# wangxb29/PPST

Hardware: AMD Instinct MI355X
Metric: 512x512 portrait swaps/sec/GPU (higher is better)
Workload: dtype bf16x3 (fp32 split into hi+lo bf16, 3 MFMA passes, fp32 accumulate); 1 GPU; simple_swapping 512x512 batch=8 per GPU, generator+encoders forward only (BASELINE configs[1]); image_parallel=1 batch per rank, no data-path collective

## Files before the change

include/ppst_hip.h:

```cpp
#ifndef PPST_HIP_H
#define PPST_HIP_H

#include <stddef.h>
#include <stdint.h>

#ifdef __cplusplus
extern "C" {
#endif

#define PPST_OK 0
#define PPST_EINVAL (-1)
#define PPST_EUNSUPPORTED (-2)
#define PPST_ENULL (-3)

enum { PPST_F32 = 0, PPST_F16 = 1, PPST_BF16 = 2, PPST_F64 = 3  };

enum { PPST_PAD_ZERO = 0, PPST_PAD_REFLECT = 1, PPST_PAD_REPLICATE = 2 };

enum { PPST_ACT_NONE = 0, PPST_ACT_LRELU = 1 , PPST_ACT_PRELU = 2 };

#define PPST_ABI_VERSION 3
int ppst_version(void);

#define PPST_ST_F32 0
// ... 73 lines not shown

typedef struct ppst_conv_args {
  const void* x;
  const void* wpack;
  const void* steps;
  void* y;
  const void* bias;
  const void* noise;
  const void* prelu;
  void* stats;
  const void* residual;
  float noise_weight;
  float out_scale;
  int32_t B, in_h, in_w, in_ld;
  int32_t out_h, out_w, out_ld, cout;
  int32_t nsteps, n_groups;
  int32_t pad_mode;
  int32_t in_off_y, in_off_x;
  int32_t out_sy, out_sx;
  int32_t act;
  int32_t precision;
  int32_t res_ld;
  int32_t tile_h, tile_w;
  int32_t halo;
  int32_t bn;
  const void* in_scale_shift;
  const void* in_prelu;
  int32_t in_c, in_act;
  int32_t flop_steps;
  int32_t tile_rows;
  int32_t a_slots;
  int32_t early_a;
  int32_t variant;
  int32_t reserved0;
  int32_t dual_b;
  int32_t io_st;
  int32_t k64;
  const void* in_res;
  int32_t in_res_ld;
  int32_t ksplit;
  const int32_t* ksplit_starts;
  void* ksplit_scratch;
  unsigned* ksplit_flags;
  uint32_t ksplit_epoch;
} ppst_conv_args;

int ppst_conv2d_mfma(const ppst_conv_args* a, void* stream);
int64_t ppst_conv_pack_wino_bytes(int cout, int cin);
int ppst_conv_pack_wino(const void* w, int64_t sn, int64_t sc, int64_t sy, int64_t sx, float scale, int cout, int cin,
                        void* out, void* stream);
int ppst_conv2d_f32(const ppst_conv_args* a, const void* w, int64_t sn, int64_t sc, int64_t sy, int64_t sx, float wscale,
                    const int32_t* src_c, const int32_t* src_ky, const int32_t* src_kx, void* stream);
int ppst_conv_tiles(int tile_h, int tile_w, int tile_rows);

int ppst_conv1x1_small_cin(const void* x, const void* w, const void* bias, void* y,
                           int64_t npix, int cin, int in_ld, int cout, float wscale,
                           int act, void* stream);
int ppst_conv1x1_small_cin_st(const void* x, const void* w, const void* bias, void* y,
                              int64_t npix, int cin, int in_ld, int cout, float wscale,
                              int act, int y_st , void* stream);
int ppst_conv1x1_small_cout(const void* x, const void* w, const void* bias, void* y,
                            int64_t npix, int cin, int cout, float wscale, void* stream);
int ppst_conv1x1_small_cout_st(const void* x, const void* w, const void* bias, void* y,
                               int64_t npix, int cin, int cout, float wscale, int x_st , void* stream);
int ppst_torgb_apply_st(const void* x, const void* scale_shift, const void* res, int res_ld, float out_scale, const void* w,
                        const void* bias, void* y, int B, int H, int W, int cin, float wscale, int x_st, void* stream);

int ppst_in_stats(const void* x, void* partial, int B, int H, int W, int C, int ld,
                  int rep_pad, int* n_partials, void* stream);
int ppst_in_finalize(const void* partial, int n_partials, const void* style,
                     int style_ld ,
                     const void* post_bias ,
                     void* scale_shift , int B, int C, double count,
                     float eps, void* stream);
int ppst_affine_act(const void* x, const void* scale_shift, const void* res,
                    const void* res_scale_shift , void* y,
                    int B, int64_t hw, int C, int x_ld, int res_ld, int y_ld,
                    int act , const void* prelu,
                    float out_scale,
                    int res_up2_w ,
                    void* stream);
int ppst_affine_act_st(const void* x, const void* scale_shift, const void* res, const void* res_scale_shift, void* y,
                       int B, int64_t hw, int C, int x_ld, int res_ld, int y_ld, int act, const void* prelu,
                       float out_scale, int res_up2_w, int x_st, int y_st, void* stream);
int ppst_affine_act_stats(const void* x, const void* scale_shift, const void* res,
                          const void* res_scale_shift, void* y, void* partial,
                          int B, int H, int W, int C, int x_ld, int res_ld, int y_ld,
                          int act, const void* prelu, float out_scale, int rep_pad,
                          int res_up2 , void* stream);
int ppst_upsample_nearest2(const void* x, void* y, int B, int H, int W, int C, void* stream);
int ppst_upsample_nearest2_st(const void* x, void* y, int B, int H, int W, int C, int st, void* stream);

int64_t ppst_gap_gmp_ws(int B, int64_t hw, int C);
int ppst_gap_gmp(const void* x, const void* mask, void* out, void* ws, int B, int H, int W,
                 int C, int ld, void* stream);
int ppst_gap_gmp_st(const void* x, const void* mask, void* out, void* ws, int B, int H, int W,
                    int C, int ld, int x_st, void* stream);
#define PPST_GROUP_MAX 32
typedef struct {
  const void* x;
  const void* mask;
  void* out;
  int32_t H, W, C, ld;
} ppst_gap_gmp_level;
int64_t ppst_gap_gmp_multi_level_ws(const ppst_gap_gmp_level* levels, int n, int B);
int ppst_gap_gmp_multi_level(const ppst_gap_gmp_level* levels, int n, int B, void* ws, int x_st, void* stream);
// ... 185 lines not shown
```

ppst_amd/_lib.py:

```python
import ctypes
import os

import torch

HERE = os.path.dirname(os.path.abspath(__file__))
LIB_PATH = os.environ.get("PPST_HIP_LIB") or os.path.join(HERE, "libppst_hip.so")

if not os.path.exists(LIB_PATH):
    raise ImportError(
        "ppst_amd: %s is missing -- build it with `python -m ppst_amd.build` "
        "(hipcc --offload-arch=gfx950). There is no CPU fallback." % LIB_PATH)

lib = ctypes.CDLL(LIB_PATH)

vp, i32, i64, f32, f64 = ctypes.c_void_p, ctypes.c_int, ctypes.c_int64, ctypes.c_float, ctypes.c_double


class PackJob(ctypes.Structure):
    _fields_ = [("w", vp), ("sn", i64), ("sc", i64), ("sy", i64), ("sx", i64), ("src_c", vp), ("src_ky", vp), ("src_kx", vp),
                ("out", vp), ("total", i64), ("block0", i64), ("scale", f32), ("cout", i32), ("bn", i32), ("nsteps", i32),
                ("n_groups", i32), ("x3", i32), ("f16", i32), ("nblocks", i32), ("dual", i32)]


class UpscaleJob(ctypes.Structure):
# ... 12 lines not shown
class LerpProblem(ctypes.Structure):
    _fields_ = [("a", vp), ("b", vp), ("y", vp), ("n", i64), ("r", f32)]


class GapGmpLevel(ctypes.Structure):
    _fields_ = [("x", vp), ("mask", vp), ("out", vp), ("H", i32), ("W", i32), ("C", i32), ("ld", i32)]


GROUP_MAX = 32


class ConvArgs(ctypes.Structure):
    _fields_ = [
        ("x", vp), ("wpack", vp), ("steps", vp), ("y", vp), ("bias", vp), ("noise", vp),
        ("prelu", vp), ("stats", vp), ("residual", vp),
        ("noise_weight", f32), ("out_scale", f32),
        ("B", i32), ("in_h", i32), ("in_w", i32), ("in_ld", i32),
        ("out_h", i32), ("out_w", i32), ("out_ld", i32), ("cout", i32),
        ("nsteps", i32), ("n_groups", i32), ("pad_mode", i32),
        ("in_off_y", i32), ("in_off_x", i32), ("out_sy", i32), ("out_sx", i32),
        ("act", i32), ("precision", i32), ("res_ld", i32), ("tile_h", i32), ("tile_w", i32),
        ("halo", i32), ("bn", i32), ("in_scale_shift", vp), ("in_prelu", vp), ("in_c", i32), ("in_act", i32),
        ("flop_steps", i32), ("tile_rows", i32), ("a_slots", i32), ("early_a", i32), ("variant", i32), ("reserved0", i32), ("dual_b", i32), ("io_st", i32), ("k64", i32),
        ("in_res", vp), ("in_res_ld", i32), ("ksplit", i32), ("ksplit_starts", vp),
        ("ksplit_scratch", vp), ("ksplit_flags", vp), ("ksplit_epoch", ctypes.c_uint32),
    ]


_SIGS = {
    "ppst_version": (i32, []),
    "ppst_guided_filter_tune": (i32, [i32, i32]),
    "ppst_upfirdn2d": (i32, [vp, vp, vp] + [i32] * 14 + [i32, vp]),
    "ppst_blur_nhwc": (i32, [vp, vp, vp] + [i32] * 10 + [vp, i32, vp]),
    "ppst_blur_nhwc_st": (i32, [vp, vp, vp] + [i32] * 10 + [vp, i32, i32, vp]),
    "ppst_fused_bias_act": (i32, [vp, vp, vp, vp, i64, i32, i32, i32, i32, f32, f32, i32, vp]),
    "ppst_nchw_to_nhwc": (i32, [vp, vp, i32, i32, i32, i32, vp]),
    "ppst_nhwc_to_nchw": (i32, [vp, vp, i32, i32, i32, i32, vp]),
    "ppst_conv_pack": (i32, [vp, i64, i64, i64, i64, f32, i32, i32, vp, vp, vp, i32, i32, i32, vp, vp]),
    "ppst_conv_pack_k64": (i32, [vp, i64, i64, i64, i64, f32, i32, i32, vp, vp, vp, i32, i32, i32, i32, vp, vp]),
    "ppst_conv_pack_up9_bytes": (i64, [i32, i32]),
    "ppst_conv_pack_up9": (i32, [vp, i64, i64, i64, i64, f32, i32, i32, vp, vp]),
    "ppst_conv_pack_wino_bytes": (i64, [i32, i32]),
    "ppst_conv_pack_wino": (i32, [vp, i64, i64, i64, i64, f32, i32, i32, vp, vp]),
    "ppst_conv_pack_dual": (i32, [vp, i64, i64, i64, i64, f32, i32, vp, vp, vp, i32, i32, i32, vp, vp]),
    "ppst_upscale_weight": (i32, [vp, vp, i32, i32, f32, vp]),
    "ppst_dgrad_s2d_stack_weight": (i32, [vp, vp, i32, i32, vp]),
    "ppst_depth_to_space_st": (i32, [vp, vp, i32, i32, i32, i32, i32, i32, i32, vp]),
    "ppst_pack_job_blocks": (i32, [i64]),
    "ppst_conv_pack_batch": (i32, [vp, i32, i32, vp]),
    "ppst_upscale_weight_batch": (i32, [vp, i32, i32, vp]),
    "ppst_conv2d_mfma": (i32, [ctypes.POINTER(ConvArgs), vp]),
    "ppst_conv2d_f32": (i32, [ctypes.POINTER(ConvArgs), vp, i64, i64, i64, i64, f32, vp, vp, vp, vp]),
    "ppst_conv_tiles": (i32, [i32, i32, i32]),
    "ppst_conv1x1_small_cin": (i32, [vp, vp, vp, vp, i64, i32, i32, i32, f32, i32, vp]),
    "ppst_conv1x1_small_cin_st": (i32, [vp, vp, vp, vp, i64, i32, i32, i32, f32, i32, i32, vp]),
    "ppst_conv1x1_small_cout": (i32, [vp, vp, vp, vp, i64, i32, i32, f32, vp]),
    "ppst_conv1x1_small_cout_st": (i32, [vp, vp, vp, vp, i64, i32, i32, f32, i32, vp]),
    "ppst_torgb_apply_st": (i32, [vp, vp, vp, i32, f32, vp, vp, vp, i32, i32, i32, i32, f32, i32, vp]),
    "ppst_in_stats": (i32, [vp, vp, i32, i32, i32, i32, i32, i32, ctypes.POINTER(i32), vp]),
    "ppst_in_finalize": (i32, [vp, i32, vp, i32, vp, vp, i32, i32, f64, f32, vp]),
    "ppst_affine_act": (i32, [vp, vp, vp, vp, vp, i32, i64, i32, i32, i32, i32, i32, vp, f32, i32, vp]),
    "ppst_affine_act_st": (i32, [vp, vp, vp, vp, vp, i32, i64, i32, i32, i32, i32, i32, vp, f32, i32, i32, i32, vp]),
    "ppst_affine_act_stats": (i32, [vp, vp, vp, vp, vp, vp, i32, i32, i32, i32, i32, i32, i32, i32, vp, f32, i32, i32, vp]),
    "ppst_upsample_nearest2": (i32, [vp, vp, i32, i32, i32, i32, vp]),
    "ppst_upsample_nearest2_st": (i32, [vp, vp, i32, i32, i32, i32, i32, vp]),
    "ppst_gap_gmp_ws": (i64, [i32, i64, i32]),
    "ppst_gap_gmp": (i32, [vp, vp, vp, vp, i32, i32, i32, i32, i32, vp]),
    "ppst_gap_gmp_st": (i32, [vp, vp, vp, vp, i32, i32, i32, i32, i32, i32, vp]),
    "ppst_avgpool": (i32, [vp, vp, i32, i32, i32, i32, i32, i32, i32, vp]),
    "ppst_bilinear": (i32, [vp, vp, i32, i32, i32, i32, i32, i32, i32, i32, vp]),
    "ppst_head_tail": (i32, [vp, vp, vp, vp, vp] + [i32] * 10 + [vp]),
    "ppst_maxpool2": (i32, [vp, vp, i32, i32, i32, i32, vp]),
    "ppst_linear": (i32, [vp, vp, vp, vp, i32, i32, i32, f32, f32, i32, i32, vp]),
    "ppst_l2norm_rows": (i32, [vp, vp, i32, i32, f32, i32, vp]),
    "ppst_lerp": (i32, [vp, vp, vp, i64, f32, vp]),
    "ppst_linear_grouped": (i32, [vp, i32, vp]),
    "ppst_l2norm_rows_grouped": (i32, [vp, i32, vp]),
    "ppst_lerp_grouped": (i32, [vp, i32, vp]),
    "ppst_gap_gmp_multi_level_ws": (i64, [vp, i32, i32]),
    "ppst_gap_gmp_multi_level": (i32, [vp, i32, i32, vp, i32, vp]),
    "ppst_spatial_modulation": (i32, [vp, vp, vp, vp, i32, i64, i32, vp]),
    "ppst_spatial_modulation_st": (i32, [vp, vp, vp, vp, i32, i64, i32, i32, vp]),
    "ppst_rselfcorr": (i32, [vp, vp, i32, i32, i32, i32, i32, vp]),
    "ppst_corr_prep": (i32, [vp, vp, i32, i32, i32, i32, vp]),
    "ppst_gemm_nt_f32": (i32, [vp, vp, vp, i32, i32, i32, i32, f32, vp]),
    "ppst_gemm_nn_f32": (i32, [vp, vp, vp, i32, i32, i32, i32, i32, i32, vp]),
    "ppst_unfold_rows": (i32, [vp, vp, i32, i32, i32, i32, i32, vp]),
    "ppst_unfold_rows_bwd": (i32, [vp, vp, i32, i32, i32, i32, i32, vp]),
    "ppst_gemm_nt_split": (i32, [vp, vp, vp, i32, i32, i32, i32, f32, i32, vp]),
    "ppst_gemm_nn_split": (i32, [vp, vp, vp, i32, i32, i32, i32, i32, i32, i32, vp]),
    "ppst_softmax_rows": (i32, [vp, i64, i32, f32, vp]),
    "ppst_unfold_patches": (i32, [vp, vp, i32, i32, i32, i32, i32, vp]),
    "ppst_fold_patches": (i32, [vp, vp, i32, i32, i32, i32, i32, vp]),
    "ppst_tensor2im_u8": (i32, [vp, vp, i32, i32, i32, i32, vp]),
    "ppst_resample_u8": (i32, [vp, vp, i32, i32, i32, i32, i32, i32, vp, vp, i32, vp]),
    "ppst_u8_to_tensor": (i32, [vp, vp, i32, i32, i32, i32, f32, f32, vp]),
    "ppst_resample_f32": (i32, [vp, vp, i32, i32, i32, i32, i32, vp, vp, i32, vp, vp, i32, i32, f32, f32, vp]),
    "ppst_png_bound": (i64, [i32, i32, i32]),
    "ppst_png_ws": (i64, [i32, i32, i32, i32]),
    "ppst_png_encode": (i32, [vp, vp, vp, i32, i32, i32, i32, vp, vp]),
    "ppst_lpips_pack_floats": (i64, []),
    "ppst_lpips_pack": (i32, [vp, vp, vp, vp, vp, vp, vp]),
    "ppst_lpips_dims": (i32, [i32, i32, ctypes.POINTER(i32)]),
    "ppst_lpips_ws": (i64, [i32, i32, i32]),
    "ppst_lpips_trunk": (i32, [vp, vp, ctypes.POINTER(i64), i32, vp, ctypes.POINTER(i64), i32, i32, i32, vp, vp]),
    "ppst_lpips_feature": (i32, [vp, i32, i32, i32, i32, vp, vp]),
# ... 89 lines not shown
```

ppst_amd/csrc/conv_wino.hip:

```cpp
#include "common.h"

struct WinoKArgs {
  const float* x;
  const unsigned char* wpack;
  const int4* steps;
  float* y;
  const float* bias;
  const float* noise;
  const float* prelu;
  float* stats;
  const float* residual;
  float noise_weight, out_scale;
  int B, in_h, in_w, in_ld, out_ld, cout, nchunk, pad_mode, act, res_ld;
  int tiles_y, tiles_x, n_tiles;
  const float* in_ss;
  const float* in_prelu;
  int in_c, in_act;
  KSplitDev ks;
};

__device__ __forceinline__ int wino_pad_index(int i, int n, int mode) {
  if (mode == PPST_PAD_REFLECT) {
    if (i < 0) i = -i;
    if (i >= n) i = 2 * (n - 1) - i;
  }
  return i < 0 ? 0 : (i >= n ? n - 1 : i);
}

#define WINO_LDA(dst, off) dst = *(const bf16x8*)(smem + (off))
#define WINO_MFMA(a_, b_, c_) c_ = __builtin_amdgcn_mfma_f32_16x16x32_bf16(a_, b_, c_, 0, 0, 0)
#define WINO_STEP_BYTES 8192
#define WINO_OOB ((int)0x80000000)

__device__ __forceinline__ void wino_split4(float4 v, uint2& hi, uint2& lo) {
  const unsigned h0 = f2bf_pk((ppst_f2){v.x, v.y}), h1 = f2bf_pk((ppst_f2){v.z, v.w});
  const float rx = v.x - __uint_as_float(h0 << 16), ry = v.y - __uint_as_float(h0 & 0xffff0000u);
  const float rz = v.z - __uint_as_float(h1 << 16), rw = v.w - __uint_as_float(h1 & 0xffff0000u);
  hi = make_uint2(h0, h1);
  lo = make_uint2(f2bf_pk((ppst_f2){rx, ry}), f2bf_pk((ppst_f2){rz, rw}));
}

__device__ __forceinline__ float wino_swap1(float v) {
  return __int_as_float(__builtin_amdgcn_update_dpp(0, __float_as_int(v), 0x128, 0xF, 0xF, true));
}

__device__ __forceinline__ int wino_lane() {
  int l = __builtin_amdgcn_mbcnt_hi(~0u, __builtin_amdgcn_mbcnt_lo(~0u, 0u));
  asm volatile("" : "+v"(l));
  return l;
}

template <int INMODE, bool KS = false>
__global__ __launch_bounds__(512, 2) void conv_wino_kernel(WinoKArgs a) {
  constexpr bool INSS = INMODE != 0;
  constexpr int NWV = 8, NTH = 64 * NWV, NTW = 4;
  constexpr int NRND = 3;
  constexpr int NP = 8, HH = 18;
  constexpr int PLANE = HH * NP * 16;
  constexpr int XIB = 8 * PLANE;
  constexpr int ABUF = 4 * XIB + 128;
  constexpr int TROW = 36;
  constexpr int TXI = 128 * TROW;
  constexpr int TBUF = 4 * TXI;
  __shared__ __attribute__((aligned(256))) unsigned char smem[2 * ABUF + 1024 * 2 * 4];
  float* const ss_lds = (float*)(smem + 2 * ABUF);

  const int nwg = gridDim.x;
  int wid;
  {
    int id = blockIdx.x, q = nwg >> 3, r = nwg & 7, xcd = id & 7;
    wid = (xcd < r ? xcd * (q + 1) : r * (q + 1) + (xcd - r) * q) + (id >> 3);
  }
  const int m_count = a.B * a.tiles_y * a.tiles_x;
  const int ntile = wid / m_count;
  int midx = wid - ntile * m_count;
  const int b = midx / (a.tiles_y * a.tiles_x);
  midx -= b * a.tiles_y * a.tiles_x;
  const int tyi = midx / a.tiles_x, txi = midx - tyi * a.tiles_x;
  const int ty0 = tyi * 16, tx0 = txi * 16;

  const int tid = threadIdx.x, lane = tid & 63, wave = __builtin_amdgcn_readfirstlane(tid >> 6);
  const int xi = wave >> 1, nh = wave & 1;
  const int r16 = lane & 15, g = lane >> 4;

#if defined(__HIP_DEVICE_COMPILE__)
  typedef const __attribute__((address_space(4))) int4* StepPtr;
#else
  typedef const int4* StepPtr;
#endif
  StepPtr steps = (StepPtr)a.steps;
  int nchunk = a.nchunk, c0 = 0;
  if (KS && a.ks.S > 1) {
    int s0, s1;
    ks_range(a.ks, (int)blockIdx.y, s0, s1);
    c0 = s0 / 9;
    nchunk = s1 / 9 - c0;
    steps += c0 * 9;
  }
  const int nsteps = nchunk * 3;
  const int64_t xoff_ = (int64_t)b * a.in_h * a.in_w * a.in_ld;
  const float* xb = a.x + (((int64_t)__builtin_amdgcn_readfirstlane((int)(xoff_ >> 32)) << 32) | (unsigned)__builtin_amdgcn_readfirstlane((int)xoff_));

  const int sp = lane & 7, se = (lane >> 3) & 1, sg = lane >> 4;
  int colA, colB;
  bool okA, okB;
  {
    auto col = [&](int k, bool& ok) __attribute__((always_inline)) {
      int ix = tx0 + 2 * sp - 1 + k;
      ok = (ix >= 0 && ix < a.in_w) || a.pad_mode != PPST_PAD_ZERO;
      ix = wino_pad_index(ix, a.in_w, a.pad_mode);
      return ok ? (ix * a.in_ld + sg * 8) * 4 : WINO_OOB;
    };
    colA = col(se ? 3 : 0, okA);
    colB = col(se ? 1 : 2, okB);
  }
  const bool interior = a.pad_mode != PPST_PAD_ZERO || (ty0 >= 1 && ty0 + 16 < a.in_h && tx0 >= 1 && tx0 + 16 < a.in_w);
  int rowoff[NRND];
#pragma unroll
  for (int r = 0; r < NRND; ++r) {
    const int hrow = wave + NWV * r;
    int iy = ty0 + hrow - 1;
    const bool inb = iy >= 0 && iy < a.in_h;
    int o = -1;
    if (hrow < HH && (inb || a.pad_mode != PPST_PAD_ZERO)) {
      iy = wino_pad_index(iy, a.in_h, a.pad_mode);
      o = iy * a.in_w * a.in_ld * 4;
    }
    rowoff[r] = __builtin_amdgcn_readfirstlane(o);
  }
  const __amdgpu_buffer_rsrc_t xrs = __builtin_amdgcn_make_buffer_rsrc((void*)xb, 0, a.in_h * a.in_w * a.in_ld * 4, 0x00020000);
  const float in_slope = (INSS && a.in_act == PPST_ACT_PRELU && a.in_prelu) ? a.in_prelu[0] : 0.f;
  const float in_neg = !INSS ? 1.f : a.in_act == PPST_ACT_LRELU ? 0.2f : a.in_act == PPST_ACT_PRELU ? in_slope : 1.f;
  const float in_pos = (INSS && a.in_act == PPST_ACT_LRELU) ? 1.41421356237309515f : 1.f;
  auto in_act = [&](float t) __attribute__((always_inline)) -> float { return (t > 0.f ? t : t * in_neg) * in_pos; };
  float4 rd[4];
  auto stage_load = [&](float4 (&q)[4], int r, int chan) __attribute__((always_inline)) {
    const int so = (rowoff[r] >= 0 ? rowoff[r] : 0) + chan * 4;
    const int va = (INMODE == 0 && rowoff[r] < 0) ? WINO_OOB : colA, vb = (INMODE == 0 && rowoff[r] < 0) ? WINO_OOB : colB;
    q[0] = __builtin_bit_cast(float4, __builtin_amdgcn_raw_buffer_load_b128(xrs, va, so, 0));
    q[1] = __builtin_bit_cast(float4, __builtin_amdgcn_raw_buffer_load_b128(xrs, va, so + 16, 0));
    q[2] = __builtin_bit_cast(float4, __builtin_amdgcn_raw_buffer_load_b128(xrs, vb, so, 0));
    q[3] = __builtin_bit_cast(float4, __builtin_amdgcn_raw_buffer_load_b128(xrs, vb, so + 16, 0));
  };
  auto stage_skip = [&](int r) __attribute__((always_inline)) { return r == NRND - 1 && wave >= 2; };
  const int chan_first = steps[0].x;
  auto stage_prep = [&](float4 (&q)[4], int r, int chan, int part) __attribute__((always_inline)) {
    const bool rowok = rowoff[r] >= 0;
    if (INSS) {
      const float4* p = (const float4*)((const unsigned char*)ss_lds + (chan - chan_first) * 8 + (wino_lane() >> 4) * 64) + part * 2;
      const float4 s0 = p[0], s1 = p[1];
      auto nact = [&](float t) __attribute__((always_inline)) -> float { return INMODE == 2 ? in_act(t) : t; };
      if (interior) {
#pragma unroll
        for (int h = part; h < 4; h += 2) {
          float4 v = q[h];
          v.x = nact(s0.x * v.x + s0.y); v.y = nact(s0.z * v.y + s0.w);
          v.z = nact(s1.x * v.z + s1.y); v.w = nact(s1.z * v.w + s1.w);
          q[h] = v;
        }
      } else {
#pragma unroll
        for (int h = part; h < 4; h += 2) {
          float4 v = q[h];
          if (rowok && (h < 2 ? okA : okB)) {
            v.x = nact(s0.x * v.x + s0.y); v.y = nact(s0.z * v.y + s0.w);
            v.z = nact(s1.x * v.z + s1.y); v.w = nact(s1.z * v.w + s1.w);
          } else v = make_float4(0.f, 0.f, 0.f, 0.f);
          q[h] = v;
        }
      }
    }
  };
  auto stage_put = [&](float4 (&q)[4], int r, int slot, int piece) __attribute__((always_inline)) {
    const int hrow = wave + NWV * r;
    const float4 A0 = q[0], A1 = q[1], B0_ = q[2], B1_ = q[3];
    float4 V0, V1;
    int i;
    const int ln = wino_lane(), se = (ln >> 3) & 1, stb = (ln >> 4) * PLANE + (ln & 7) * 16;
    const float sgn = se ? -1.f : 1.f;
    if (piece == 0) {
      i = se ? 3 : 0;
      V0 = make_float4(A0.x - B0_.x, A0.y - B0_.y, A0.z - B0_.z, A0.w - B0_.w);
      V1 = make_float4(A1.x - B1_.x, A1.y - B1_.y, A1.z - B1_.z, A1.w - B1_.w);
    } else {
      i = se ? 2 : 1;
      V0 = make_float4(wino_swap1(B0_.x) + sgn * B0_.x, wino_swap1(B0_.y) + sgn * B0_.y, wino_swap1(B0_.z) + sgn * B0_.z, wino_swap1(B0_.w) + sgn * B0_.w);
      V1 = make_float4(wino_swap1(B1_.x) + sgn * B1_.x, wino_swap1(B1_.y) + sgn * B1_.y, wino_swap1(B1_.z) + sgn * B1_.z, wino_swap1(B1_.w) + sgn * B1_.w);
    }
    uint2 h0, l0, h1, l1;
    wino_split4(V0, h0, l0);
    wino_split4(V1, h1, l1);
    unsigned char* dst = smem + (slot * ABUF + hrow * NP * 16) + i * XIB + stb;
    *(uint4*)dst = make_uint4(h0.x, h0.y, h1.x, h1.y);
    *(uint4*)(dst + 4 * PLANE) = make_uint4(l0.x, l0.y, l1.x, l1.y);
  };

  const int64_t woff_ = ((((int64_t)ntile * 4 + xi) * 2 + nh) * (a.nchunk * 3) + c0 * 3) * WINO_STEP_BYTES;
  const unsigned char* wbase = a.wpack + (((int64_t)__builtin_amdgcn_readfirstlane((int)(woff_ >> 32)) << 32) |
                                          (unsigned)__builtin_amdgcn_readfirstlane((int)woff_));
  const __amdgpu_buffer_rsrc_t wrs = __builtin_amdgcn_make_buffer_rsrc((void*)wbase, 0, nsteps * WINO_STEP_BYTES, 0x00020000);
  bf16x8 B0[2][2], B1[2][2];
  auto load_b = [&](bf16x8 (&dst)[2][2], int s, int half) __attribute__((always_inline)) {
    const int so = s * WINO_STEP_BYTES + half * 4096;
    const int lo16 = wino_lane() * 16;
#pragma unroll
    for (int n = 0; n < 2; ++n)
#pragma unroll
      for (int h = 0; h < 2; ++h)
        dst[n][h] = __builtin_bit_cast(bf16x8, __builtin_amdgcn_raw_buffer_load_b128(wrs, lo16 + (n * 2 + h) * 1024, so, 0));
  };

  load_b(B0, 0, 0); load_b(B1, 0, 1);
  {
    float4 q[NRND][4];
#pragma unroll
    for (int r = 0; r < NRND; ++r) stage_load(q[r], r, chan_first);
    if (INSS) {
      const float* src = a.in_ss + ((int64_t)b * a.in_c + chan_first) * 2;
      for (int i = tid * 4; i < nchunk * 64; i += NTH * 4) *(float4*)(ss_lds + i) = *(const float4*)(src + i);
      __syncthreads();
    }
#pragma unroll
    for (int r = 0; r < NRND; ++r) {
      if (!stage_skip(r)) {
        stage_prep(q[r], r, chan_first, 0); stage_prep(q[r], r, chan_first, 1);
        stage_put(q[r], r, 0, 0); stage_put(q[r], r, 0, 1);
      }
    }
  }
  asm volatile("s_waitcnt lgkmcnt(0)\n\ts_barrier" ::: "memory");

  f32x4 acc[8][NTW];
#pragma unroll
  for (int i = 0; i < 8; ++i)
#pragma unroll
    for (int j = 0; j < NTW; ++j) acc[i][j] = (f32x4){0.f, 0.f, 0.f, 0.f};

#define WA_OFF(slot, dy, mt) ((slot) * ABUF + xi * XIB + g * PLANE + ((2 * (mt) + (dy)) * NP + r16) * 16)
  int s = 0;
  for (int c = 0; c < nchunk; ++c) {
    const int slot = c & 1;
    const bool more = c + 1 < nchunk;
    const int chan_next = steps[(more ? c + 1 : c) * 9].x;
    const int aoff0 = WA_OFF(slot, 0, 0);
    int aoff1 = aoff0;
    asm volatile("" : "+v"(aoff1));
    bf16x8 ah = *(const bf16x8*)(smem + aoff0);
    bf16x8 al = *(const bf16x8*)(smem + aoff0 + 4 * PLANE);
#pragma unroll
    for (int dy = 0; dy < 3; ++dy) {
      const int sn = s + 1 < nsteps ? s + 1 : s;
      stage_load(rd, dy, chan_next);
      __builtin_amdgcn_sched_barrier(0);
#pragma unroll
      for (int mt = 0; mt < 8; ++mt) {
        bf16x8 nh_, nl_;
        if (mt < 7) {
          WINO_LDA(nh_, aoff0 + (2 * (mt + 1) + dy) * NP * 16);
          WINO_LDA(nl_, aoff0 + (2 * (mt + 1) + dy) * NP * 16 + 4 * PLANE);
        } else {
          WINO_LDA(nh_, aoff1 + dy * NP * 16);
          WINO_LDA(nl_, aoff1 + dy * NP * 16 + 4 * PLANE);
        }
        __builtin_amdgcn_sched_barrier(0);
#pragma unroll
        for (int n = 0; n < 2; ++n) {
          WINO_MFMA(al, B0[n][0], acc[mt][n]);
          WINO_MFMA(ah, B0[n][1], acc[mt][n]);
          WINO_MFMA(ah, B0[n][0], acc[mt][n]);
        }
        ah = nh_;
        al = nl_;
      }
      __builtin_amdgcn_sched_barrier(0);
      load_b(B0, sn, 0);
      __builtin_amdgcn_sched_barrier(0);
      const bool skip = stage_skip(dy);
#pragma unroll
      for (int mt = 0; mt < 8; ++mt) {
        bf16x8 nh_ = ah, nl_ = al;
        if (mt < 7) {
          WINO_LDA(nh_, aoff1 + (2 * (mt + 1) + dy) * NP * 16);
          WINO_LDA(nl_, aoff1 + (2 * (mt + 1) + dy) * NP * 16 + 4 * PLANE);
        } else if (dy < 2) {
          WINO_LDA(nh_, aoff0 + (dy + 1) * NP * 16);
          WINO_LDA(nl_, aoff0 + (dy + 1) * NP * 16 + 4 * PLANE);
        }
        __builtin_amdgcn_sched_barrier(0);
        if (!skip) {
          if (mt == 2) stage_prep(rd, dy, chan_next, 0);
          if (mt == 3) stage_prep(rd, dy, chan_next, 1);
          if (mt == 4) stage_put(rd, dy, slot ^ 1, 0);
          if (mt == 6) stage_put(rd, dy, slot ^ 1, 1);
        }
#pragma unroll
        for (int n = 0; n < 2; ++n) {
          WINO_MFMA(al, B1[n][0], acc[mt][2 + n]);
          WINO_MFMA(ah, B1[n][1], acc[mt][2 + n]);
          WINO_MFMA(ah, B1[n][0], acc[mt][2 + n]);
        }
        ah = nh_;
        al = nl_;
      }
      __builtin_amdgcn_sched_barrier(0);
      load_b(B1, sn, 1);
      __builtin_amdgcn_sched_barrier(0);
      ++s;
    }
    asm volatile("s_waitcnt lgkmcnt(0)\n\ts_barrier" ::: "memory");
  }
#undef WA_OFF

  if (KS && a.ks.S > 1) {
    const int S = a.ks.S, y = (int)blockIdx.y;
    float* const slot0 = a.ks.scratch + (int64_t)wid * (S - 1) * (8 * NTW * 4 * NTH) + tid;
    if (y < S - 1) {
      float* const dst = slot0 + (int64_t)y * (8 * NTW * 4 * NTH);
      KS_SCATTER(acc, 8, NTW, NTH, dst)
      ks_publish(a.ks, wid, y, tid);
      return;
    }
    ks_wait(a.ks, wid, tid);
    KS_GATHER(acc, 8, NTW, NTH, S, slot0);
  }

  float* const T = (float*)smem;
  float* const red = (float*)smem;
  const int act = a.act & 0xff;
  const bool res_after = (a.act >> 8) & 1;
  const float slope = (act == PPST_ACT_PRELU && a.prelu) ? a.prelu[0] : 0.f;
  constexpr int NML = NTH / 32, NIT = 32 / NML;
  const int f32_ = tid & 31, mloc = tid >> 5;
  const int n0 = ntile * 128 + f32_ * 4;
  const bool nok = n0 < a.cout;
  const int64_t img = (int64_t)b * a.in_h * a.in_w;
  float* const yb = a.y + img * a.out_ld;
  const float* const nzb = a.noise ? a.noise + img : nullptr;
  const float* const rb = a.residual ? a.residual + img * a.res_ld : nullptr;
  const float4 bv = __builtin_bit_cast(float4, __builtin_amdgcn_raw_buffer_load_b128(__builtin_amdgcn_make_buffer_rsrc((void*)(a.bias ? (const void*)a.bias : (const void*)a.y), 0, a.bias ? a.cout * 4 : 0, 0x00020000), n0 * 4, 0, 0));
  float nzv[8 * NIT];
  {
    const __amdgpu_buffer_rsrc_t nrs = __builtin_amdgcn_make_buffer_rsrc((void*)(nzb ? nzb : (const float*)yb), 0,
                                                                         nzb ? a.in_h * a.in_w * 4 : 0, 0x00020000);
#pragma unroll
    for (int i = 0; i < 8 * NIT; ++i) {
      const int m = 32 * (i / (2 * NIT)) + NML * ((i >> 1) % NIT) + mloc;
      const int oy = ty0 + (m >> 3), ox = tx0 + 2 * (m & 7) + (i & 1);
      nzv[i] = a.noise_weight * __builtin_bit_cast(float, __builtin_amdgcn_raw_buffer_load_b32(
                                    nrs, (oy < a.in_h && ox < a.in_w) ? (oy * a.in_w + ox) * 4 : WINO_OOB, 0, 0));
    }
  }
  float4 s1a = make_float4(0.f, 0.f, 0.f, 0.f), s2a = s1a;
  const int resm = a.residual ? (res_after ? 2 : 1) : 0;
  constexpr int TROW2 = 132, TXI2 = 32 * TROW2, TBUF2 = 4 * TXI2;
  auto epi_passes = [&](auto act_c) __attribute__((always_inline)) {
#pragma clang fp contract(off)
    const int ACT = act_c.value;
#pragma unroll
    for (int ph = 0; ph < 4; ++ph) {
      float* tw = T + (ph & 1) * TBUF2 + xi * TXI2 + nh * 64 + r16;
#pragma unroll
      for (int ml = 0; ml < 2; ++ml)
#pragma unroll
        for (int nt = 0; nt < NTW; ++nt)
#pragma unroll
          for (int j = 0; j < 4; ++j) tw[(ml * 16 + g * 4 + j) * TROW2 + nt * 16] = acc[ph * 2 + ml][nt][j];
      asm volatile("s_waitcnt lgkmcnt(0)\n\ts_barrier" ::: "memory");
      const float* tr = T + (ph & 1) * TBUF2 + f32_ * 4;
#pragma unroll
      for (int it = 0; it < NIT; ++it) {
        const int ml_ = it * NML + mloc, m = ph * 32 + ml_;
        const float4 v0 = *(const float4*)(tr + 0 * TXI2 + ml_ * TROW2), v1 = *(const float4*)(tr + 1 * TXI2 + ml_ * TROW2);
        const float4 v2 = *(const float4*)(tr + 2 * TXI2 + ml_ * TROW2), v3 = *(const float4*)(tr + 3 * TXI2 + ml_ * TROW2);
        const int oy = ty0 + (m >> 3), ox0 = tx0 + 2 * (m & 7);
#pragma unroll
        for (int px = 0; px < 2; ++px) {
          if (nok && oy < a.in_h && ox0 + px < a.in_w) {
            float o[4];
            if (px == 0) { o[0] = (v0.x + v1.x) + v2.x; o[1] = (v0.y + v1.y) + v2.y; o[2] = (v0.z + v1.z) + v2.z; o[3] = (v0.w + v1.w) + v2.w; }
            else         { o[0] = (v1.x - v2.x) + v3.x; o[1] = (v1.y - v2.y) + v3.y; o[2] = (v1.z - v2.z) + v3.z; o[3] = (v1.w - v2.w) + v3.w; }
            const int pix = oy * a.in_w + ox0 + px;
            const float nz = nzv[ph * 2 * NIT + it * 2 + px];
            float4 rv = make_float4(0.f, 0.f, 0.f, 0.f);
            if (resm) rv = *(const float4*)(rb + (pix * a.res_ld + n0));
            const float r4[4] = {rv.x, rv.y, rv.z, rv.w};
            const float b4[4] = {bv.x, bv.y, bv.z, bv.w};
#pragma unroll
            for (int cc = 0; cc < 4; ++cc) {
              float t = o[cc] + b4[cc] + nz;
              if (resm == 1) t += r4[cc];
              if (ACT == PPST_ACT_LRELU) t = (t > 0.f ? t : t * 0.2f) * 1.41421356237309515f;
              else if (ACT == PPST_ACT_PRELU) t = t >= 0.f ? t : t * slope;
              if (resm == 2) t += r4[cc];
              o[cc] = t * a.out_scale;
            }
            PPST_EPI_STORE(yb + (pix * a.out_ld + n0), o);
            s1a.x += o[0]; s1a.y += o[1]; s1a.z += o[2]; s1a.w += o[3];
            s2a.x += o[0] * o[0]; s2a.y += o[1] * o[1]; s2a.z += o[2] * o[2]; s2a.w += o[3] * o[3];
          }
        }
      }
    }
  };
  if (act == PPST_ACT_LRELU) epi_passes(EpiC<PPST_ACT_LRELU>{});
  else if (act == PPST_ACT_PRELU) epi_passes(EpiC<PPST_ACT_PRELU>{});
  else epi_passes(EpiC<PPST_ACT_NONE>{});

  if (a.stats) {
    float4 s1 = s1a, s2 = s2a;
    s1.x += __shfl_xor(s1.x, 32, 64); s1.y += __shfl_xor(s1.y, 32, 64); s1.z += __shfl_xor(s1.z, 32, 64); s1.w += __shfl_xor(s1.w, 32, 64);
    s2.x += __shfl_xor(s2.x, 32, 64); s2.y += __shfl_xor(s2.y, 32, 64); s2.z += __shfl_xor(s2.z, 32, 64); s2.w += __shfl_xor(s2.w, 32, 64);
    __syncthreads();
    if (lane < 32) {
      float* r = red + (wave * 128 + f32_ * 4) * 2;
      r[0] = s1.x; r[1] = s2.x; r[2] = s1.y; r[3] = s2.y; r[4] = s1.z; r[5] = s2.z; r[6] = s1.w; r[7] = s2.w;
    }
    __syncthreads();
    if (tid < 128) {
      const int n = ntile * 128 + tid;
      if (n < a.cout) {
        float t0 = 0.f, t1 = 0.f;
#pragma unroll
        for (int w = 0; w < NWV; ++w) { t0 += red[(w * 128 + tid) * 2]; t1 += red[(w * 128 + tid) * 2 + 1]; }
        float* o = a.stats + ((((int64_t)b * a.tiles_y + tyi) * a.tiles_x + txi) * a.cout + n) * 2;
        o[0] = t0;
        o[1] = t1;
      }
    }
  }
}

int ppst_conv_wino_launch(const ppst_conv_args* a, int n_tiles, int tiles_y, int tiles_x, hipStream_t st) {
  WinoKArgs k;
  k.x = (const float*)a->x; k.wpack = (const unsigned char*)a->wpack; k.steps = (const int4*)a->steps; k.y = (float*)a->y;
  k.bias = (const float*)a->bias; k.noise = (const float*)a->noise; k.prelu = (const float*)a->prelu;
  k.stats = (float*)a->stats; k.residual = (const float*)a->residual;
  k.noise_weight = a->noise_weight; k.out_scale = a->out_scale;
  k.B = a->B; k.in_h = a->in_h; k.in_w = a->in_w; k.in_ld = a->in_ld; k.out_ld = a->out_ld; k.cout = a->cout;
  k.nchunk = a->nsteps / 9; k.pad_mode = a->pad_mode; k.act = a->act; k.res_ld = a->res_ld;
  k.tiles_y = tiles_y; k.tiles_x = tiles_x; k.n_tiles = n_tiles;
  k.in_ss = (const float*)a->in_scale_shift; k.in_prelu = (const float*)a->in_prelu;
  k.in_c = a->in_c; k.in_act = a->in_act;
  const int blocks = n_tiles * a->B * tiles_y * tiles_x;
  k.ks.scratch = nullptr; k.ks.flags = nullptr; k.ks.epoch = 0; k.ks.S = 1;
  if (a->ksplit > 1) {
    if (!a->ksplit_starts && k.nchunk % a->ksplit) return PPST_EINVAL;
    const int e0 = ppst_ksplit_prepare_(a, blocks, 128, 512, &k.ks);
    if (e0 != PPST_OK) return e0;
    for (int i = 1; i < a->ksplit; ++i)
      if (k.ks.start[i] % 9) return PPST_EINVAL;
  }
  if (k.ks.S > 1) {
    const dim3 gridk(blocks, k.ks.S);
    if (k.in_ss && k.in_act != PPST_ACT_NONE) PPST_LAUNCH((conv_wino_kernel<2, true>), gridk, dim3(512), 0, st, k);
    else if (k.in_ss) PPST_LAUNCH((conv_wino_kernel<1, true>), gridk, dim3(512), 0, st, k);
    else PPST_LAUNCH((conv_wino_kernel<0, true>), gridk, dim3(512), 0, st, k);
    return PPST_LAUNCH_CHECK();
  }
  const dim3 grid(blocks);
  if (k.in_ss && k.in_act != PPST_ACT_NONE) PPST_LAUNCH((conv_wino_kernel<2>), grid, dim3(512), 0, st, k);
  else if (k.in_ss) PPST_LAUNCH((conv_wino_kernel<1>), grid, dim3(512), 0, st, k);
  else PPST_LAUNCH((conv_wino_kernel<0>), grid, dim3(512), 0, st, k);
  return PPST_LAUNCH_CHECK();
}

struct WinoPackJob {
  const float* w;
  int64_t sn, sc, sy, sx;
  unsigned short* out;
  int64_t total;
  float scale;
  int cout, nchunk;
};
__global__ __launch_bounds__(256) void conv_pack_wino_kernel(WinoPackJob j) {
  for (int64_t t = (int64_t)blockIdx.x * 256 + threadIdx.x; t < j.total; t += (int64_t)gridDim.x * 256) {
    const int lane = (int)(t & 63);
    int64_t r = t >> 6;
    const int ntq = (int)(r & 3); r >>= 2;
    const int ky = (int)(r % 3); r /= 3;
    const int c = (int)(r % j.nchunk); r /= j.nchunk;
    const int nh = (int)(r & 1); r >>= 1;
    const int xi = (int)(r & 3);
    const int ntile = (int)(r >> 2);
    const int n = ntile * 128 + nh * 64 + ntq * 16 + (lane & 15);
    const int c0 = c * 32 + (lane >> 4) * 8;
    unsigned short hi[8], lo[8];
#pragma unroll
    for (int q = 0; q < 8; ++q) {
      double u = 0.0;
      if (n < j.cout) {
        const float* wp = j.w + n * j.sn + (int64_t)(c0 + q) * j.sc + ky * j.sy;
        const double g0 = (double)wp[0] * (double)j.scale, g1 = (double)wp[j.sx] * (double)j.scale, g2 = (double)wp[2 * j.sx] * (double)j.scale;
        u = xi == 0 ? g0 : xi == 1 ? 0.5 * (g0 + g1 + g2) : xi == 2 ? 0.5 * (g0 - g1 + g2) : g2;
      }
      const float uf = (float)u;
      hi[q] = f2bf(uf);
      lo[q] = f2bf((float)(u - (double)bf2f(hi[q])));
    }
    unsigned short* oh = j.out + (((t >> 6) * 2) * 64 + lane) * 8;
#pragma unroll
    for (int q = 0; q < 8; ++q) oh[q] = hi[q];
#pragma unroll
    for (int q = 0; q < 8; ++q) oh[64 * 8 + q] = lo[q];
  }
}
extern "C" int64_t ppst_conv_pack_wino_bytes(int cout, int cin) {
  if (cout <= 0 || cin <= 0 || cin % 32) return 0;
  return (int64_t)cdiv(cout, 128) * 8 * (cin / 32) * 3 * WINO_STEP_BYTES;
}
extern "C" int ppst_conv_pack_wino(const void* w, int64_t sn, int64_t sc, int64_t sy, int64_t sx, float scale, int cout, int cin,
                                   void* out, void* stream) {
  if (cout <= 0 || cin <= 0 || cin % 32) return PPST_EINVAL;
// ... 11 lines not shown
```

Before: 164.6 swaps/s (all GPUs).

## Make Winograd conv kernel persistent with cross-tile prefetch of next tile's input

Turns the non-split Winograd conv kernel into a persistent kernel. The grid is capped at the CU count and each workgroup walks a contiguous run of tiles, assigned XCD-aware. When consecutive tiles share the same output-channel tile and image, the next tile's first input chunk and weights are prefetched during the last chunk of the current one, and the double-buffer parity is carried over. This is meant to remove launch and prologue cost per tile and overlap staging with compute. In exchange the epilogue runs from a single LDS buffer with extra barriers, and occupancy is limited to one workgroup per CU even though launch bounds allow two.

```diff
diff --git a/include/ppst_hip.h b/include/ppst_hip.h
--- a/include/ppst_hip.h
+++ b/include/ppst_hip.h
@@ -149,6 +149,7 @@
 int ppst_conv2d_f32(const ppst_conv_args* a, const void* w, int64_t sn, int64_t sc, int64_t sy, int64_t sx, float wscale,
                     const int32_t* src_c, const int32_t* src_ky, const int32_t* src_kx, void* stream);
 int ppst_conv_tiles(int tile_h, int tile_w, int tile_rows);
+int ppst_conv_wino_tile_run(int tiles, int grid, int block, int* first, int* count);
 
 int ppst_conv1x1_small_cin(const void* x, const void* w, const void* bias, void* y,
                            int64_t npix, int cin, int in_ld, int cout, float wscale,
diff --git a/ppst_amd/_lib.py b/ppst_amd/_lib.py
--- a/ppst_amd/_lib.py
+++ b/ppst_amd/_lib.py
@@ -88,6 +88,7 @@
     "ppst_conv2d_mfma": (i32, [ctypes.POINTER(ConvArgs), vp]),
     "ppst_conv2d_f32": (i32, [ctypes.POINTER(ConvArgs), vp, i64, i64, i64, i64, f32, vp, vp, vp, vp]),
     "ppst_conv_tiles": (i32, [i32, i32, i32]),
+    "ppst_conv_wino_tile_run": (i32, [i32, i32, i32, ctypes.POINTER(i32), ctypes.POINTER(i32)]),
     "ppst_conv1x1_small_cin": (i32, [vp, vp, vp, vp, i64, i32, i32, i32, f32, i32, vp]),
     "ppst_conv1x1_small_cin_st": (i32, [vp, vp, vp, vp, i64, i32, i32, i32, f32, i32, i32, vp]),
     "ppst_conv1x1_small_cout": (i32, [vp, vp, vp, vp, i64, i32, i32, f32, vp]),
diff --git a/ppst_amd/csrc/conv_wino.hip b/ppst_amd/csrc/conv_wino.hip
--- a/ppst_amd/csrc/conv_wino.hip
+++ b/ppst_amd/csrc/conv_wino.hip
@@ -50,6 +50,16 @@
   return l;
 }
 
+__host__ __device__ __forceinline__ void wino_tile_run(int tiles, int nwg, int id, int& first, int& count) {
+  const int xcd = id & 7, j = id >> 3;
+  const int q = tiles >> 3, r = tiles & 7;
+  const int start = xcd < r ? xcd * (q + 1) : r * (q + 1) + (xcd - r) * q, cnt = q + (xcd < r ? 1 : 0);
+  const int nb = (nwg >> 3) + (xcd < (nwg & 7) ? 1 : 0);
+  const int len = cnt / nb, rem = cnt - len * nb;
+  first = start + j * len + (j < rem ? j : rem);
+  count = len + (j < rem ? 1 : 0);
+}
+
 template <int INMODE, bool KS = false>
 __global__ __launch_bounds__(512, 2) void conv_wino_kernel(WinoKArgs a) {
   constexpr bool INSS = INMODE != 0;
@@ -65,19 +75,30 @@
   __shared__ __attribute__((aligned(256))) unsigned char smem[2 * ABUF + 1024 * 2 * 4];
   float* const ss_lds = (float*)(smem + 2 * ABUF);
 
+  constexpr bool PERS = !KS;
   const int nwg = gridDim.x;
-  int wid;
-  {
+  const int m_img = a.tiles_y * a.tiles_x, m_count = a.B * m_img;
+  int wid, t_end;
+  if (PERS) {
+    int n_;
+    wino_tile_run(a.n_tiles * m_count, nwg, (int)blockIdx.x, wid, n_);
+    t_end = wid + n_;
+    if (n_ <= 0) return;
+  } else {
     int id = blockIdx.x, q = nwg >> 3, r = nwg & 7, xcd = id & 7;
     wid = (xcd < r ? xcd * (q + 1) : r * (q + 1) + (xcd - r) * q) + (id >> 3);
-  }
-  const int m_count = a.B * a.tiles_y * a.tiles_x;
-  const int ntile = wid / m_count;
-  int midx = wid - ntile * m_count;
-  const int b = midx / (a.tiles_y * a.tiles_x);
-  midx -= b * a.tiles_y * a.tiles_x;
-  const int tyi = midx / a.tiles_x, txi = midx - tyi * a.tiles_x;
-  const int ty0 = tyi * 16, tx0 = txi * 16;
+    t_end = wid + 1;
+  }
+  auto decode = [&](int t, int& nt_, int& b_, int& ty_, int& tx_) __attribute__((always_inline)) {
+    nt_ = t / m_count;
+    int m = t - nt_ * m_count;
+    b_ = m / m_img;
+    m -= b_ * m_img;
+    ty_ = m / a.tiles_x;
+    tx_ = m - ty_ * a.tiles_x;
+  };
+  int ntile, b, tyi, txi;
+  decode(wid, ntile, b, tyi, txi);
 
   const int tid = threadIdx.x, lane = tid & 63, wave = __builtin_amdgcn_readfirstlane(tid >> 6);
   const int xi = wave >> 1, nh = wave & 1;
@@ -98,13 +119,14 @@
     steps += c0 * 9;
   }
   const int nsteps = nchunk * 3;
-  const int64_t xoff_ = (int64_t)b * a.in_h * a.in_w * a.in_ld;
-  const float* xb = a.x + (((int64_t)__builtin_amdgcn_readfirstlane((int)(xoff_ >> 32)) << 32) | (unsigned)__builtin_amdgcn_readfirstlane((int)xoff_));
-
-  const int sp = lane & 7, se = (lane >> 3) & 1, sg = lane >> 4;
+
   int colA, colB;
   bool okA, okB;
-  {
+  bool interior;
+  int rowoff[NRND];
+  auto set_tile = [&](int ty0, int tx0) __attribute__((always_inline)) {
+    const int ln = PERS ? wino_lane() : lane;
+    const int sp = ln & 7, se = (ln >> 3) & 1, sg = ln >> 4;
     auto col = [&](int k, bool& ok) __attribute__((always_inline)) {
       int ix = tx0 + 2 * sp - 1 + k;
       ok = (ix >= 0 && ix < a.in_w) || a.pad_mode != PPST_PAD_ZERO;
@@ -113,22 +135,26 @@
     };
     colA = col(se ? 3 : 0, okA);
     colB = col(se ? 1 : 2, okB);
-  }
-  const bool interior = a.pad_mode != PPST_PAD_ZERO || (ty0 >= 1 && ty0 + 16 < a.in_h && tx0 >= 1 && tx0 + 16 < a.in_w);
-  int rowoff[NRND];
-#pragma unroll
-  for (int r = 0; r < NRND; ++r) {
-    const int hrow = wave + NWV * r;
-    int iy = ty0 + hrow - 1;
-    const bool inb = iy >= 0 && iy < a.in_h;
-    int o = -1;
-    if (hrow < HH && (inb || a.pad_mode != PPST_PAD_ZERO)) {
-      iy = wino_pad_index(iy, a.in_h, a.pad_mode);
-      o = iy * a.in_w * a.in_ld * 4;
-    }
-    rowoff[r] = __builtin_amdgcn_readfirstlane(o);
-  }
-  const __amdgpu_buffer_rsrc_t xrs = __builtin_amdgcn_make_buffer_rsrc((void*)xb, 0, a.in_h * a.in_w * a.in_ld * 4, 0x00020000);
+    interior = a.pad_mode != PPST_PAD_ZERO || (ty0 >= 1 && ty0 + 16 < a.in_h && tx0 >= 1 && tx0 + 16 < a.in_w);
+#pragma unroll
+    for (int r = 0; r < NRND; ++r) {
+      const int hrow = wave + NWV * r;
+      int iy = ty0 + hrow - 1;
+      const bool inb = iy >= 0 && iy < a.in_h;
+      int o = -1;
+      if (hrow < HH && (inb || a.pad_mode != PPST_PAD_ZERO)) {
+        iy = wino_pad_index(iy, a.in_h, a.pad_mode);
+        o = iy * a.in_w * a.in_ld * 4;
+      }
+      rowoff[r] = __builtin_amdgcn_readfirstlane(o);
+    }
+  };
+  __amdgpu_buffer_rsrc_t xrs;
+  auto set_image = [&](int b_) __attribute__((always_inline)) {
+    const int64_t xoff_ = (int64_t)b_ * a.in_h * a.in_w * a.in_ld;
+    const float* xb = a.x + (((int64_t)__builtin_amdgcn_readfirstlane((int)(xoff_ >> 32)) << 32) | (unsigned)__builtin_amdgcn_readfirstlane((int)xoff_));
+    xrs = __builtin_amdgcn_make_buffer_rsrc((void*)xb, 0, a.in_h * a.in_w * a.in_ld * 4, 0x00020000);
+  };
   const float in_slope = (INSS && a.in_act == PPST_ACT_PRELU && a.in_prelu) ? a.in_prelu[0] : 0.f;
   const float in_neg = !INSS ? 1.f : a.in_act == PPST_ACT_LRELU ? 0.2f : a.in_act == PPST_ACT_PRELU ? in_slope : 1.f;
   const float in_pos = (INSS && a.in_act == PPST_ACT_LRELU) ? 1.41421356237309515f : 1.f;
@@ -195,10 +221,13 @@
     *(uint4*)(dst + 4 * PLANE) = make_uint4(l0.x, l0.y, l1.x, l1.y);
   };
 
-  const int64_t woff_ = ((((int64_t)ntile * 4 + xi) * 2 + nh) * (a.nchunk * 3) + c0 * 3) * WINO_STEP_BYTES;
-  const unsigned char* wbase = a.wpack + (((int64_t)__builtin_amdgcn_readfirstlane((int)(woff_ >> 32)) << 32) |
-                                          (unsigned)__builtin_amdgcn_readfirstlane((int)woff_));
-  const __amdgpu_buffer_rsrc_t wrs = __builtin_amdgcn_make_buffer_rsrc((void*)wbase, 0, nsteps * WINO_STEP_BYTES, 0x00020000);
+  __amdgpu_buffer_rsrc_t wrs;
+  auto set_ntile = [&](int nt_) __attribute__((always_inline)) {
+    const int64_t woff_ = ((((int64_t)nt_ * 4 + xi) * 2 + nh) * (a.nchunk * 3) + c0 * 3) * WINO_STEP_BYTES;
+    const unsigned char* wbase = a.wpack + (((int64_t)__builtin_amdgcn_readfirstlane((int)(woff_ >> 32)) << 32) |
+                                            (unsigned)__builtin_amdgcn_readfirstlane((int)woff_));
+    wrs = __builtin_amdgcn_make_buffer_rsrc((void*)wbase, 0, nsteps * WINO_STEP_BYTES, 0x00020000);
+  };
   bf16x8 B0[2][2], B1[2][2];
   auto load_b = [&](bf16x8 (&dst)[2][2], int s, int half) __attribute__((always_inline)) {
     const int so = s * WINO_STEP_BYTES + half * 4096;
@@ -210,8 +239,21 @@
         dst[n][h] = __builtin_bit_cast(bf16x8, __builtin_amdgcn_raw_buffer_load_b128(wrs, lo16 + (n * 2 + h) * 1024, so, 0));
   };
 
-  load_b(B0, 0, 0); load_b(B1, 0, 1);
-  {
+  int par = 0;
+  bool staged = false;
+  for (;;) {
+  const int ty0 = tyi * 16, tx0 = txi * 16;
+  int ntile_n = ntile, b_n = b, tyi_n = tyi, txi_n = txi;
+  bool pipe = false;
+  if (PERS && wid + 1 < t_end) {
+    decode(wid + 1, ntile_n, b_n, tyi_n, txi_n);
+    pipe = ntile_n == ntile && b_n == b;
+  }
+  if (!PERS || !staged) {
+    set_image(b);
+    set_ntile(ntile);
+    set_tile(ty0, tx0);
+    load_b(B0, 0, 0); load_b(B1, 0, 1);
     float4 q[NRND][4];
 #pragma unroll
     for (int r = 0; r < NRND; ++r) stage_load(q[r], r, chan_first);
@@ -224,11 +266,11 @@
     for (int r = 0; r < NRND; ++r) {
       if (!stage_skip(r)) {
         stage_prep(q[r], r, chan_first, 0); stage_prep(q[r], r, chan_first, 1);
-        stage_put(q[r], r, 0, 0); stage_put(q[r], r, 0, 1);
-      }
-    }
-  }
-  asm volatile("s_waitcnt lgkmcnt(0)\n\ts_barrier" ::: "memory");
+        stage_put(q[r], r, par, 0); stage_put(q[r], r, par, 1);
+      }
+    }
+    asm volatile("s_waitcnt lgkmcnt(0)\n\ts_barrier" ::: "memory");
+  }
 
   f32x4 acc[8][NTW];
 #pragma unroll
@@ -239,9 +281,11 @@
 #define WA_OFF(slot, dy, mt) ((slot) * ABUF + xi * XIB + g * PLANE + ((2 * (mt) + (dy)) * NP + r16) * 16)
   int s = 0;
   for (int c = 0; c < nchunk; ++c) {
-    const int slot = c & 1;
+    const int slot = (par + c) & 1;
     const bool more = c + 1 < nchunk;
-    const int chan_next = steps[(more ? c + 1 : c) * 9].x;
+    const bool ahead = PERS && pipe && !more;
+    if (ahead) set_tile(tyi_n * 16, txi_n * 16);
+    const int chan_next = steps[(more ? c + 1 : ahead ? 0 : c) * 9].x;
     const int aoff0 = WA_OFF(slot, 0, 0);
     int aoff1 = aoff0;
     asm volatile("" : "+v"(aoff1));
@@ -249,7 +293,7 @@
     bf16x8 al = *(const bf16x8*)(smem + aoff0 + 4 * PLANE);
 #pragma unroll
     for (int dy = 0; dy < 3; ++dy) {
-      const int sn = s + 1 < nsteps ? s + 1 : s;
+      const int sn = s + 1 < nsteps ? s + 1 : (PERS && pipe) ? 0 : s;
       stage_load(rd, dy, chan_next);
       __builtin_amdgcn_sched_barrier(0);
 #pragma unroll
@@ -324,13 +368,16 @@
     KS_GATHER(acc, 8, NTW, NTH, S, slot0);
   }
 
-  float* const T = (float*)smem;
-  float* const red = (float*)smem;
+  const bool one_buf = PERS && pipe;
+  float* const T = (float*)(smem + (one_buf ? ((par + nchunk - 1) & 1) * ABUF : 0));
+  float* const red = T;
   const int act = a.act & 0xff;
   const bool res_after = (a.act >> 8) & 1;
   const float slope = (act == PPST_ACT_PRELU && a.prelu) ? a.prelu[0] : 0.f;
   constexpr int NML = NTH / 32, NIT = 32 / NML;
-  const int f32_ = tid & 31, mloc = tid >> 5;
+  int tid_e = tid;
+  if (PERS) asm volatile("" : "+v"(tid_e));
+  const int f32_ = tid_e & 31, mloc = tid_e >> 5;
   const int n0 = ntile * 128 + f32_ * 4;
   const bool nok = n0 < a.cout;
   const int64_t img = (int64_t)b * a.in_h * a.in_w;
@@ -358,7 +405,8 @@
     const int ACT = act_c.value;
 #pragma unroll
     for (int ph = 0; ph < 4; ++ph) {
-      float* tw = T + (ph & 1) * TBUF2 + xi * TXI2 + nh * 64 + r16;
+      if (one_buf && ph > 0) asm volatile("s_waitcnt lgkmcnt(0)\n\ts_barrier" ::: "memory");
+      float* tw = T + (one_buf ? 0 : (ph & 1) * TBUF2) + xi * TXI2 + nh * 64 + r16;
 #pragma unroll
       for (int ml = 0; ml < 2; ++ml)
 #pragma unroll
@@ -366,7 +414,7 @@
 #pragma unroll
           for (int j = 0; j < 4; ++j) tw[(ml * 16 + g * 4 + j) * TROW2 + nt * 16] = acc[ph * 2 + ml][nt][j];
       asm volatile("s_waitcnt lgkmcnt(0)\n\ts_barrier" ::: "memory");
-      const float* tr = T + (ph & 1) * TBUF2 + f32_ * 4;
+      const float* tr = T + (one_buf ? 0 : (ph & 1) * TBUF2) + f32_ * 4;
 #pragma unroll
       for (int it = 0; it < NIT; ++it) {
         const int ml_ = it * NML + mloc, m = ph * 32 + ml_;
@@ -410,12 +458,12 @@
     float4 s1 = s1a, s2 = s2a;
     s1.x += __shfl_xor(s1.x, 32, 64); s1.y += __shfl_xor(s1.y, 32, 64); s1.z += __shfl_xor(s1.z, 32, 64); s1.w += __shfl_xor(s1.w, 32, 64);
     s2.x += __shfl_xor(s2.x, 32, 64); s2.y += __shfl_xor(s2.y, 32, 64); s2.z += __shfl_xor(s2.z, 32, 64); s2.w += __shfl_xor(s2.w, 32, 64);
-    __syncthreads();
+    if (PERS) asm volatile("s_waitcnt lgkmcnt(0)\n\ts_barrier" ::: "memory"); else __syncthreads();
     if (lane < 32) {
       float* r = red + (wave * 128 + f32_ * 4) * 2;
       r[0] = s1.x; r[1] = s2.x; r[2] = s1.y; r[3] = s2.y; r[4] = s1.z; r[5] = s2.z; r[6] = s1.w; r[7] = s2.w;
     }
-    __syncthreads();
+    if (PERS) asm volatile("s_waitcnt lgkmcnt(0)\n\ts_barrier" ::: "memory"); else __syncthreads();
     if (tid < 128) {
       const int n = ntile * 128 + tid;
       if (n < a.cout) {
@@ -428,6 +476,31 @@
       }
     }
   }
+  if (!PERS || ++wid >= t_end) break;
+  asm volatile("s_waitcnt lgkmcnt(0)\n\ts_barrier" ::: "memory");
+  par = (par + nchunk) & 1;
+  staged = pipe;
+  ntile = ntile_n; b = b_n; tyi = tyi_n; txi = txi_n;
+  }
+}
+
+static int wino_cu_count() {
+  static int cached[64];
+  int dev = 0;
+  if (hipGetDevice(&dev) != hipSuccess || dev < 0 || dev >= 64) return 0;
+  int n = cached[dev];
+  if (n == 0) {
+    if (hipDeviceGetAttribute(&n, hipDeviceAttributeMultiprocessorCount, dev) != hipSuccess || n <= 0) return 0;
+    cached[dev] = n = n < 8 ? 8 : n;
+  }
+  return n;
+}
+
+extern "C" int ppst_conv_wino_tile_run(int tiles, int grid, int block, int* first, int* count) {
+  if (!first || !count) return PPST_ENULL;
+  if (tiles <= 0 || grid <= 0 || grid > tiles || (grid < 8 && grid != tiles) || block < 0 || block >= grid) return PPST_EINVAL;
+  wino_tile_run(tiles, grid, block, *first, *count);
+  return PPST_OK;
 }
 
 int ppst_conv_wino_launch(const ppst_conv_args* a, int n_tiles, int tiles_y, int tiles_x, hipStream_t st) {
@@ -457,7 +530,9 @@
     else PPST_LAUNCH((conv_wino_kernel<0, true>), gridk, dim3(512), 0, st, k);
     return PPST_LAUNCH_CHECK();
   }
-  const dim3 grid(blocks);
+  const int cus = wino_cu_count();
+  if (cus <= 0) return PPST_EINVAL;
+  const dim3 grid(blocks < cus ? blocks : cus);
   if (k.in_ss && k.in_act != PPST_ACT_NONE) PPST_LAUNCH((conv_wino_kernel<2>), grid, dim3(512), 0, st, k);
   else if (k.in_ss) PPST_LAUNCH((conv_wino_kernel<1>), grid, dim3(512), 0, st, k);
   else PPST_LAUNCH((conv_wino_kernel<0>), grid, dim3(512), 0, st, k);
```

After: 164.1 swaps/s (all GPUs). No clear change (-0.3%).
